# 1069066484/PanoSwinTransformerObjectDetection

Hardware: AMD Instinct MI355X
Metric: panoramas/sec PanoSwin-T 512x1024 fwd+bwd (higher is better)
Workload: dtype bf16; 1 GPU; PanoSwin-T backbone (embed 96, depths 2-2-6-2, heads 3-6-12-24, ape, pano mode) fwd+bwd+AdamW on 3x512x1024 panoramas, BASELINE.json configs[1]; batch_per_gpu=8, global_batch=8, parallelism=dp1, hip_graph=True, overlap_allreduce=False, fused_window_attention=True, device=AMD Radeon Graphics

## Files before the change

include/pswin.h:

```cpp
#ifndef PSWIN_H_
#define PSWIN_H_

#include <stdint.h>

#ifdef __cplusplus
extern "C" {
#endif

#define PSWIN_ABI_VERSION 10

#define PSWIN_F32 0
#define PSWIN_BF16 1

#define PSWIN_MODE_PLANAR 0
#define PSWIN_MODE_PANO 1

#define PSWIN_OK 0
#define PSWIN_ERR_ARG (-1)
#define PSWIN_ERR_UNSUPPORTED (-2)

#define PSWIN_WS 7
#define PSWIN_WTOK 49
#define PSWIN_WPAD 64
#define PSWIN_HEAD_DIM 32

int pswin_version(void);


int pswin_window_grid(int mode, int H, int W, int* Hp, int* Wp, int* n_windows);

int pswin_window_map(int mode, int H, int W, int shift, int32_t* map, int32_t* inv, void* stream);

int pswin_planar_mask(int H, int W, int shift, float* mask, void* stream);


int pswin_uv_grid(int H, int W, float* uv, void* stream);

int pswin_abs_pos_features(const float* uv, int n, float* feat, void* stream);

int pswin_gather_uv(const float* uv, const int32_t* map, int n_slots, float* uv_win, void* stream);

int pswin_haversine_windows(const float* uv1, const float* uv2, int n_windows, float* dist, void* stream);
// ... 259 lines not shown
                              int P, int C, void* stream);



int pswin_attn_pad_tiles(const float* src, int n, int transpose, float* dst, void* stream);

int pswin_attn_fwd(const void* q, const void* k, const void* v, int ld_qkv, const float* dist_tiles, int n_dist,
                   const float* alpha, const float* beta, const float* mask_tiles, int n_mask, void* out, int ld_out,
                   float* lse, int n_chunks, int n_windows, int n_bias_windows, int heads, float scale, int dtype,
                   void* stream);

int pswin_attn_suggest_chunks(int n_windows, int n_bias_windows, int heads, int backward);

int pswin_win_attn_fused_supported(int C, int heads, int dtype);
int pswin_win_attn_fused_fwd(const void* x, const void* w_qkv, const float* b_qkv, const void* w_proj, const float* dist_tiles,
                             int n_dist, const float* alpha, const float* beta, const float* mask_tiles, int n_mask, void* y,
                             void* qkv_out, void* att_out, float* lse_out, long long n_windows, int n_bias_windows, int C,
                             int heads, float scale, int dtype, void* stream);

int pswin_qkv_attn_fused_supported(int C, int heads, int dtype);
int pswin_qkv_attn_fused_fwd(const void* x, const void* w_qkv, const float* b_qkv, const float* dist_tiles, int n_dist, const float* alpha,
                             const float* beta, const float* mask_tiles, int n_mask, void* y, void* qkv_out, float* lse_out, long long n_windows,
                             int n_bias_windows, int C, int heads, float scale, int dtype, void* stream);

int pswin_attn_bwd(const void* q, const void* k, const void* v, int ld_qkv, const float* dist_tiles_t, int n_dist,
                   const float* alpha, const float* beta, const float* mask_tiles_t, int n_mask, const void* dout,
                   int ld_out, const float* lse, void* dq, void* dk, void* dv, int ld_dqkv, float* dscore_sum,
                   int n_chunks, int n_windows, int n_bias_windows, int heads, float scale, int dtype, void* stream);
int pswin_attn_bwd_ex(const void* q, const void* k, const void* v, int ld_qkv, long long qkv_window_stride, int qkv_head_stride,
                      const float* dist_tiles_t, int n_dist, const float* alpha, const float* beta, const float* mask_tiles_t,
                      int n_mask, const void* dout, int ld_out, const float* lse, void* dq, void* dk, void* dv, int ld_dqkv,
                      float* dscore_sum, int n_chunks, int n_windows, int n_bias_windows, int heads, float scale, int dtype,
                      void* stream);


int pswin_attn_table_grads_workspace(int heads);
int pswin_attn_table_grads_partial_rows(int n_tiles, int heads);
int pswin_attn_table_grads(const float* dscore_sum, int n_tiles, int n_bias_windows, const float* dist_tiles_t,
                           int n_dist, int heads, float* dalpha, float* dbeta, float* workspace, void* stream);

typedef struct pswin_table_grad_job {
    const float* dscore_sum;
    const float* dist_tiles_t;
    float* dalpha;
    float* dbeta;
    float* workspace;
    int n_tiles;
    int n_bias_windows;
    int n_dist;
    int heads;
} pswin_table_grad_job;
int pswin_attn_table_grads_batch(const pswin_table_grad_job* jobs, int n_jobs, int stages, void* stream);


int pswin_pano_warp_u8(const uint8_t* src, const double* params, uint8_t* dst, int B, int H, int W, int C, void* stream);

int pswin_pano_resize_normalize_pad(const uint8_t* src, const int32_t* out_hw, const float* norm, int to_rgb, float* dst, int B, int H,
                                    int W, int Hp, int Wp, void* stream);

int pswin_pano_resize_crop_resize_normalize_pad(const uint8_t* src, const int32_t* plan, const float* norm, int to_rgb, float* dst, int B,
                                                int H, int W, int Hp, int Wp, void* stream);

int pswin_pano_masks(const uint8_t* src, const double* params, const int32_t* plan, const int32_t* rows, const int32_t* count, uint8_t* dst,
                     int B, int Gin, int Gmax, int H, int W, int Hp, int Wp, void* stream);


// ... 138 lines not shown
```

panoswintransformerobjectdetection_amd/_lib.py:

```python
import ctypes
import os

import torch

_PKG = os.path.dirname(os.path.abspath(__file__))
LIB_PATH = os.environ.get("PSWIN_LIB") or os.path.join(_PKG, "libpswin_hip.so")

F32, BF16 = 0, 1
MODE_PLANAR, MODE_PANO = 0, 1
WS, WTOK, WPAD, HEAD_DIM = 7, 49, 64, 32
ABI_VERSION = 10

_vp, _i, _f = ctypes.c_void_p, ctypes.c_int, ctypes.c_float
_ip = ctypes.POINTER(ctypes.c_int)

_PROTOTYPES = {
    "pswin_version": [],
    "pswin_window_grid": [_i, _i, _i, _ip, _ip, _ip],
    "pswin_window_map": [_i, _i, _i, _i, _vp, _vp, _vp],
    "pswin_planar_mask": [_i, _i, _i, _vp, _vp],
    "pswin_uv_grid": [_i, _i, _vp, _vp],
    "pswin_abs_pos_features": [_vp, _i, _vp, _vp],
    "pswin_gather_uv": [_vp, _vp, _i, _vp, _vp],
    "pswin_haversine_windows": [_vp, _vp, _i, _vp, _vp],
    "pswin_window_gather": [_vp, _i, _vp, _vp, _vp, _i, _i, _i, _i, _i, _vp],
    "pswin_window_scatter_add": [_vp, _i, _vp, _vp, _vp, _vp, _vp, _i, _i, _i, _i, _i, _vp],
    "pswin_ln_gather_fwd": [_vp, _i, _vp, _vp, _vp, _f, _vp, _i, _vp, _vp, _i, _i, _i, _i, _vp],
    "pswin_ln_gather_fwd_add": [_vp, _i, _vp, _vp, _vp, _f, _vp, _vp, _i, _vp, _vp, _i, _i, _i, _i, _vp],
    "pswin_ln_gather_bwd": [_vp, _i, _vp, _vp, _i, _vp, _vp, _vp, _vp, _vp, _vp, _vp, _vp, _vp, _vp, _i, _i, _i, _i, _vp],
    "pswin_ln_gather_bwd_ex": [_vp, _i, _vp, _vp, _i, _vp, _vp, _vp, _vp, _vp, _vp, _vp, _vp, _vp, _vp, _i, _i, _i, _i, _vp, _vp, _i, _vp, _vp, _i,
                               _vp],
    "pswin_scatter_add_ln_fwd": [_vp, _i, _vp, _vp, _vp, _vp, _vp, _vp, _vp, _f, _vp, _i, _vp, _vp, _i, _i, _i, _i, _vp],
    "pswin_scatter_add_ln_fwd_map": [_vp, _i, _vp, _vp, _vp, _vp, _vp, _vp, _vp, _f, _vp, _i, _vp, _vp, _i, _i, _i, _i, _vp, _i, _vp, _i, _vp],
    "pswin_ln_nchw_supported": [_i, _i],
    "pswin_ln_nchw_fwd": [_vp, _vp, _vp, _f, _vp, _vp, _vp, _i, _i, _i, _vp],
    "pswin_ln_nchw_bwd": [_vp, _vp, _vp, _vp, _vp, _vp, _vp, _vp, _vp, _vp, _i, _i, _i, _vp],
    "pswin_scatter_add_ln_nchw_fwd": [_vp, _vp, _vp, _vp, _vp, _vp, _vp, _f, _vp, _vp, _vp, _i, _i, _i, _vp],
    "pswin_ln_nchw_bwd_ex": [_vp, _vp, _vp, _vp, _vp, _vp, _vp, _vp, _vp, _vp, _vp, _vp, _i, _i, _i, _vp],
    "pswin_ln_workspace": [ctypes.c_longlong, _i],
    "pswin_ln_patch_merge_fwd": [_vp, _i, _vp, _vp, _f, _vp, _i, _vp, _vp, _i, _i, _i, _i, _vp],
    "pswin_ln_patch_merge_bwd": [_vp, _i, _vp, _i, _vp, _vp, _vp, _vp, _vp, _vp, _vp, _i, _i, _i, _i, _vp],
    "pswin_patch_merge_gather": [_vp, _i, _vp, _i, _i, _i, _i, _i, _vp],
    "pswin_patch_merge_scatter": [_vp, _i, _vp, _i, _i, _i, _i, _i, _vp],
    "pswin_bn_workspace": [_i],
# ... 100 lines not shown
    "pswin_mlp0_fwd": [_vp, _vp, _vp, _vp, _vp, _vp, ctypes.c_longlong, _i, _i, _vp],
    "pswin_mlp0_bwd_supported": [_i, _i],
    "pswin_mlp0_bwd_partial_rows": [ctypes.c_longlong],
    "pswin_mlp0_bwd": [_vp, _vp, _vp, _vp, _vp, _vp, _vp, _vp, ctypes.c_longlong, _i, _i, _vp],
    "pswin_fc1_gelu_bwd": [_vp, _vp, _vp, _vp, _vp, _vp, _vp, ctypes.c_longlong, _i, _i, _vp],
    "pswin_bias_gelu_fwd": [_vp, _i, _vp, _vp, ctypes.c_longlong, _i, _vp],
    "pswin_bias_gelu_workspace": [ctypes.c_longlong, _i],
    "pswin_bias_gelu_tune": [_i, _i],
    "pswin_bias_gelu_bwd": [_vp, _vp, _i, _vp, _vp, _vp, _vp, ctypes.c_longlong, _i, _vp],
    "pswin_colsum_workspace": [ctypes.c_longlong, _i, _i],
    "pswin_colsum": [_vp, _i, ctypes.c_longlong, _i, _vp, _vp, _vp],
    "pswin_colsum_skip": [_vp, _i, ctypes.c_longlong, _i, _i, _i, _vp, _vp],
    "pswin_reduce_jobs": [_vp, _i, _vp],
    "pswin_attn_table_grads_batch": [_vp, _i, _i, _vp],
    "pswin_attn_table_grads_partial_rows": [_i, _i],
    "pswin_ln_partial_rows": [ctypes.c_longlong, _i],
    "pswin_ln_rows_tune": [_i],
    "pswin_bias_gelu_partial_rows": [ctypes.c_longlong, _i, _i],
    "pswin_fc1_gelu_partial_rows": [ctypes.c_longlong],
    "pswin_interp_rows": [_vp, _vp, _vp, _vp, _i, _i, _i, _i, _vp],
    "pswin_interp_rows_adjoint": [_vp, _vp, _vp, _vp, _i, _i, _i, _i, _vp],
    "pswin_attn_pad_tiles": [_vp, _i, _i, _vp, _vp],
    "pswin_attn_fwd": [_vp, _vp, _vp, _i, _vp, _i, _vp, _vp, _vp, _i, _vp, _i, _vp, _i, _i, _i, _i, _f, _i, _vp],
    "pswin_win_attn_fused_supported": [_i, _i, _i],
    "pswin_win_attn_fused_fwd": [_vp, _vp, _vp, _vp, _vp, _i, _vp, _vp, _vp, _i, _vp, _vp, _vp, _vp, ctypes.c_longlong, _i, _i, _i,
                                 _f, _i, _vp],
    "pswin_qkv_attn_fused_supported": [_i, _i, _i],
    "pswin_qkv_attn_fused_fwd": [_vp, _vp, _vp, _vp, _i, _vp, _vp, _vp, _i, _vp, _vp, _vp, ctypes.c_longlong, _i, _i, _i, _f, _i, _vp],
    "pswin_attn_suggest_chunks": [_i, _i, _i, _i],
    "pswin_attn_bwd": [_vp, _vp, _vp, _i, _vp, _i, _vp, _vp, _vp, _i, _vp, _i, _vp, _vp, _vp, _vp, _i, _vp,
                       _i, _i, _i, _i, _f, _i, _vp],
    "pswin_attn_bwd_ex": [_vp, _vp, _vp, _i, ctypes.c_longlong, _i, _vp, _i, _vp, _vp, _vp, _i, _vp, _i, _vp, _vp, _vp, _vp, _i, _vp,
                          _i, _i, _i, _i, _f, _i, _vp],
    "pswin_attn_table_grads_workspace": [_i],
    "pswin_attn_table_grads": [_vp, _i, _i, _vp, _i, _i, _vp, _vp, _vp, _vp],
    "pswin_pano_warp_u8": [_vp, _vp, _vp, _i, _i, _i, _i, _vp],
    "pswin_pano_resize_normalize_pad": [_vp, _vp, _vp, _i, _vp, _i, _i, _i, _i, _i, _vp],
    "pswin_pano_resize_crop_resize_normalize_pad": [_vp, _vp, _vp, _i, _vp, _i, _i, _i, _i, _i, _vp],
    "pswin_pano_masks": [_vp, _vp, _vp, _vp, _vp, _vp, _i, _i, _i, _i, _i, _i, _i, _vp],
}

_lib = None


class PswinError(RuntimeError):
    pass


class ReduceJob(ctypes.Structure):
    _fields_ = [("src", ctypes.c_void_p), ("dst", ctypes.c_void_p), ("dtype", ctypes.c_int), ("rows", ctypes.c_int),
                ("cols", ctypes.c_int), ("ld", ctypes.c_int)]


class TnJob(ctypes.Structure):
    _fields_ = [("dy", ctypes.c_void_p), ("x", ctypes.c_void_p), ("partial", ctypes.c_void_p), ("dbias_partial", ctypes.c_void_p),
                ("M", ctypes.c_longlong), ("N", ctypes.c_int), ("K", ctypes.c_int), ("splits", ctypes.c_int), ("partial_dtype", ctypes.c_int),
                ("zero_lo", ctypes.c_int), ("zero_hi", ctypes.c_int), ("sample_scale", ctypes.c_void_p), ("rows_per_sample", ctypes.c_int)]


class TransposeJob(ctypes.Structure):
    _fields_ = [("src", ctypes.c_void_p), ("dst", ctypes.c_void_p), ("rows", ctypes.c_int), ("cols", ctypes.c_int)]


class LrSchedule(ctypes.Structure):
    _fields_ = [("policy", ctypes.c_int), ("warmup", ctypes.c_int), ("warmup_iters", ctypes.c_int), ("by_epoch", ctypes.c_int),
                ("iters_per_epoch", ctypes.c_int), ("n_milestones", ctypes.c_int), ("step_every", ctypes.c_int), ("has_min_lr", ctypes.c_int),
# ... 136 lines not shown
```

panoswintransformerobjectdetection_amd/csrc/pswin_attn.hip:

```cpp
#include <cstdlib>
#include <type_traits>

#include "pswin_attn_frag.hpp"

using namespace pswin;

namespace {

struct AttnArgs {
    const void *q, *k, *v;
    const float* dist;
    const float* mask;
    const float* alpha;
    const float* beta;
    void* out;
    const void* dout;
    float* lse;
#ifdef PSWIN_ATTN_STAMPS
    unsigned long long* stamps;
#endif
    void *dq, *dk, *dv;
    float* dtab;
    int n_dist, n_mask;
    int ld_qkv, ld_out, ld_dqkv;
    long long qkv_win_stride;
    int qkv_head_stride;
    int nb, heads, reps_per_chunk, n_items;
    float scale;
};


struct TabRaw {
    float b[3], a[3];
};
static_assert(NBINS <= 3 * 64, "three table entries per lane");
__device__ inline TabRaw tables_fetch(const AttnArgs& a, int h, int lane) {
    const __amdgpu_buffer_rsrc_t bres = __builtin_amdgcn_make_buffer_rsrc(const_cast<float*>(a.beta), 0, NBINS * a.heads * 4, 0x00020000);
    const __amdgpu_buffer_rsrc_t ares = __builtin_amdgcn_make_buffer_rsrc(const_cast<float*>(a.alpha), 0, a.dist ? NBINS * a.heads * 4 : 0, 0x00020000);
    TabRaw r;
#pragma unroll
    for (int k = 0; k < 3; ++k) {
        const int off = ((lane + 64 * k) * a.heads + h) * 4;
        r.b[k] = __builtin_bit_cast(float, __builtin_amdgcn_raw_buffer_load_b32(bres, off, 0, 0));
        r.a[k] = __builtin_bit_cast(float, __builtin_amdgcn_raw_buffer_load_b32(ares, off, 0, 0));
    }
    return r;
}
__device__ inline void tables_store(const TabRaw& r, int lane, float* tab_a, float* tab_b) {
#pragma unroll
    for (int k = 0; k < 3; ++k) {
        const int t = lane + 64 * k;
        if (t < NBINS) {
            tab_b[t] = r.b[k];
            tab_a[t] = r.a[k];
        }
// ... 332 lines not shown
            for (int dt = 0; dt < 2; ++dt) kt[dt] = lds_read_tr<DT, HD>(kimg, 32 * s + 4 * g, 16 * dt, c, g);
#pragma unroll
            for (int ti = 0; ti < 4; ++ti) {
                const Frag<DT> tf = lds_read_tr<DT, PADT>(timg, 32 * s + 4 * g, 16 * ti, c, g);
#pragma unroll
                for (int dt = 0; dt < 2; ++dt) dq[dt][ti] = mma32<DT>(kt[dt], tf, dq[dt][ti]);
            }
        }
#pragma unroll
        for (int ti = 0; ti < 4; ++ti) {
            store_row8_at<DT>(window_rsrc<DT>(a.dq, dhead0, a.ld_dqkv), dx_off[ti], g, dq[0][ti] * a.scale, dq[1][ti] * a.scale);
        }
        if constexpr (DUAL) {
            if (r + 1 < a.reps_per_chunk) cur = nxt;
        }
    }
    if (a.dtab) {
        float* gt = a.dtab + (size_t)item * (PADT * PADT);
#pragma unroll
        for (int ti = 0; ti < 4; ++ti)
#pragma unroll
            for (int tj = 0; tj < 4; ++tj)
                *reinterpret_cast<f32x4*>(gt + (16 * tj + c) * PADT + 16 * ti + 4 * g) = gsum[ti][tj];
    }
}

struct PairLds {
    static constexpr int KIMG = 64 * 64;
    static constexpr int HALF = 32 * 64;
    static constexpr int TIMG = 64 * 64;
    static constexpr int EXCH = 64 * 128;
    static constexpr int TAB = 2 * TABP * 4;
    static constexpr int BYTES = KIMG + 2 * (2 * HALF + TIMG) + 2 * EXCH + TAB;
};

__device__ inline int timg_off(int row, int unit8) {
    return row * 64 + ((unit8 ^ (((row >> 1) & 1) | (((row >> 3) & 1) << 1) | (((row >> 2) & 1) << 2))) << 3);
}
__device__ inline int exch_off(int row, int chunk16) { return row * 128 + ((chunk16 ^ (row & 7)) << 4); }

template <bool TIMG>
__device__ inline Frag<PSWIN_BF16> tr32(const char* img, int R0, int col0, int c) {
    const int q = c >> 2, p = c & 3;
    typedef __attribute__((address_space(3))) s16x4* lds_s16x4_ptr;
    const int k8 = (col0 >> 2) + p;
    const char* a0 = img + (TIMG ? timg_off(R0 + q, k8) : img32_off(R0 + q, k8 >> 1) + ((k8 & 1) << 3));
    const char* a1 = a0 + 16 * 64;
    s16x4 lo = __builtin_amdgcn_ds_read_tr16_b64_v4i16((lds_s16x4_ptr)(a0));
    s16x4 hi = __builtin_amdgcn_ds_read_tr16_b64_v4i16((lds_s16x4_ptr)(a1));
    typedef __attribute__((ext_vector_type(8))) short s16x8;
    s16x8 both = {lo[0], lo[1], lo[2], lo[3], hi[0], hi[1], hi[2], hi[3]};
    Frag<PSWIN_BF16> f;
    f.v = __builtin_bit_cast(bf16x8, both);
    return f;
}

#ifdef PSWIN_ATTN_STAMPS
#define PSWIN_STAMP(i)                                                  \
    do {                                                                \
        const unsigned long long t_ = __builtin_amdgcn_s_memtime();     \
        stamp_acc[i] += t_ - stamp_last;                                \
        stamp_last = t_;                                                \
    } while (0)
#else
#define PSWIN_STAMP(i)
#endif
__global__ __launch_bounds__(128, 2) void attn_bwd_pair_kernel(AttnArgs a) {
    constexpr int DT = PSWIN_BF16;
#ifdef PSWIN_ATTN_STAMPS
    unsigned long long stamp_acc[8] = {0, 0, 0, 0, 0, 0, 0, 0}, stamp_last = __builtin_amdgcn_s_memtime();
#endif
    __shared__ __attribute__((aligned(16))) char smem[PairLds::BYTES];
    const int w = __builtin_amdgcn_readfirstlane(threadIdx.x >> 6), lane = threadIdx.x & 63;
    const int c = lane & 15, g = lane >> 4;
    const int item = blockIdx.x;
    const int h = item % a.heads;
    const int wb = (item / a.heads) % a.nb;
    const int chunk = item / (a.heads * a.nb);
    char* kimg = smem;
    char* qimg = kimg + PairLds::KIMG + w * (2 * PairLds::HALF + PairLds::TIMG);
    char* doimg = qimg + PairLds::HALF;
    char* timg = doimg + PairLds::HALF;
    float* exch_dk = reinterpret_cast<float*>(smem + PairLds::KIMG + 2 * (2 * PairLds::HALF + PairLds::TIMG));
    float* exch_dv = exch_dk + 64 * 32;
    float* tab_a = exch_dv + 64 * 32;
    float* tab_b = tab_a + TABP;
    const float* dtile = a.dist ? a.dist + (size_t)(wb % a.n_dist) * (PADT * PADT) : nullptr;
// ... 174 lines not shown
            for (int tt = 0; tt < 2; ++tt) dq[dt][tt] = f32x4{0.f, 0.f, 0.f, 0.f};
#pragma unroll
        for (int s = 0; s < 2; ++s) {
            Frag<DT> kt[2];
#pragma unroll
            for (int dt = 0; dt < 2; ++dt) kt[dt] = tr32<false>(kimg, 32 * s + 4 * g, 16 * dt, c);
#pragma unroll
            for (int tt = 0; tt < 2; ++tt) {
                const Frag<DT> tf = tr32<true>(timg, 32 * s + 4 * g, 16 * tt, c);
#pragma unroll
                for (int dt = 0; dt < 2; ++dt) dq[dt][tt] = mma32<DT>(kt[dt], tf, dq[dt][tt]);
            }
        }
#pragma unroll
        for (int tt = 0; tt < 2; ++tt) {
            store_row8_at<DT>(window_rsrc<DT>(a.dq, dhead0, a.ld_dqkv), dq_off[tt], g, dq[0][tt] * a.scale, dq[1][tt] * a.scale);
        }
        PSWIN_STAMP(5);
        __syncthreads();
        PSWIN_STAMP(6);
    }
#ifdef PSWIN_ATTN_STAMPS
    if (a.stamps && lane == 0)
        for (int i = 0; i < 8; ++i) a.stamps[((size_t)blockIdx.x * 2 + w) * 8 + i] = stamp_acc[i];
#endif
    if (a.dtab) {
        float* gt = a.dtab + (size_t)item * (PADT * PADT);
#pragma unroll
        for (int tt = 0; tt < 2; ++tt)
#pragma unroll
            for (int tj = 0; tj < 4; ++tj)
                *reinterpret_cast<f32x4*>(gt + (16 * tj + c) * PADT + 16 * (2 * w + tt) + 4 * g) = gsum[tt][tj];
    }
}

__global__ void pad_tiles_kernel(const float* __restrict__ src, int n, int transpose, float* __restrict__ dst) {
    const size_t t = blockIdx.x;
    for (int e = threadIdx.x; e < PADT * PADT; e += blockDim.x) {
        const int r = e / PADT, col = e - r * PADT;
        float v = 0.f;
        if (r < TOK && col < TOK) v = transpose ? src[(t * TOK + col) * TOK + r] : src[(t * TOK + r) * TOK + col];
        dst[t * PADT * PADT + e] = v;
    }
}

constexpr int DTAB_BLOCKS = 128;
__host__ __device__ inline int dtab_ld(int heads) { return (heads * 2 * TOK * TOK + 3) & ~3; }
inline int dtab_blocks(int n_tiles, int heads) {
    int nb = (512 + heads - 1) / heads;
    if (nb > DTAB_BLOCKS) nb = DTAB_BLOCKS;
    if (nb < 16) nb = 16;
    return n_tiles < nb ? n_tiles : nb;
}
constexpr int DTAB_THREADS = 256;

constexpr int TJ_MAX = 32;
struct TJob {
    const float* g;
    const float* dist_t;
    float* partial;
    float* summed;
    float* dalpha;
    float* dbeta;
    int n_tiles, nb, n_dist, heads, blocks;
    int first1, first2;
};
// ... 137 lines not shown
    a.nb = n_bias_windows; a.heads = heads; a.reps_per_chunk = reps / chunks;
    a.scale = scale;
    constexpr int W = 4;
    if (dtype == PSWIN_BF16) {
        a.n_items = chunks * n_bias_windows * heads * 2;
        hipLaunchKernelGGL((attn_fwd_kernel<PSWIN_BF16, W, 2>), dim3((a.n_items + W - 1) / W), dim3(64 * W), 0,
                           (hipStream_t)stream, a);
    } else {
        a.n_items = chunks * n_bias_windows * heads;
        hipLaunchKernelGGL((attn_fwd_kernel<PSWIN_F32, W, 4>), dim3((a.n_items + W - 1) / W), dim3(64 * W), 0,
                           (hipStream_t)stream, a);
    }
    PSWIN_LAUNCH_RET();
}

extern "C" int pswin_attn_suggest_chunks(int n_windows, int n_bias_windows, int heads, int backward) {
    if (n_windows <= 0 || n_bias_windows <= 0 || heads <= 0 || n_windows % n_bias_windows) return PSWIN_ERR_ARG;
    return pick_chunks(n_windows / n_bias_windows, n_bias_windows, heads, backward != 0);
}

extern "C" int pswin_attn_table_grads_partial_rows(int n_tiles, int heads) {
    return (n_tiles > 0 && heads > 0) ? dtab_blocks(n_tiles, heads) : PSWIN_ERR_ARG;
}

extern "C" int pswin_attn_table_grads_workspace(int heads) {
    return heads > 0 ? (DTAB_BLOCKS + 1) * dtab_ld(heads) : PSWIN_ERR_ARG;
}

#ifdef PSWIN_ATTN_STAMPS
static unsigned long long* g_attn_stamps = nullptr;
extern "C" void pswin_attn_debug_stamps(unsigned long long* p) { g_attn_stamps = p; }
#endif

extern "C" int pswin_attn_bwd_ex(const void* q, const void* k, const void* v, int ld_qkv, long long qkv_window_stride,
                                 int qkv_head_stride, const float* dist_t, int n_dist, const float* alpha, const float* beta,
                                 const float* mask_t, int n_mask, const void* dout, int ld_out, const float* lse, void* dq, void* dk,
                                 void* dv, int ld_dqkv, float* dscore_sum, int n_chunks, int n_windows, int n_bias_windows,
                                 int heads, float scale, int dtype, void* stream) {
    PSWIN_CHECK_ARG(q && k && v && beta && valid_dtype(dtype) && n_windows > 0 && n_bias_windows > 0 && heads > 0);
    PSWIN_CHECK_ARG(n_windows % n_bias_windows == 0 && ld_qkv >= HD && ld_qkv % 8 == 0 && qkv_head_stride % 8 == 0 && qkv_window_stride % 8 == 0);
    PSWIN_CHECK_ARG(qkv_head_stride >= HD && qkv_window_stride >= (long long)(TOK - 1) * ld_qkv + HD);
    PSWIN_CHECK_ARG(aligned16(q) && aligned16(k) && aligned16(v) && aligned16(dist_t) && aligned16(mask_t));
    PSWIN_CHECK_ARG((long long)n_windows * qkv_window_stride < (1ll << 40));
    PSWIN_CHECK_ARG(!dist_t || (alpha && n_dist > 0 && n_bias_windows % n_dist == 0));
    PSWIN_CHECK_ARG(!mask_t || (n_mask > 0 && n_bias_windows % n_mask == 0));
    PSWIN_CHECK_ARG(dout && lse && dq && dk && dv);
    PSWIN_CHECK_ARG(aligned16(dout) && aligned16(dq) && aligned16(dk) && aligned16(dv) && aligned16(lse));
    PSWIN_CHECK_ARG(ld_out >= heads * HD && ld_out % 8 == 0 && ld_dqkv >= heads * HD && ld_dqkv % 8 == 0);
    const int reps = n_windows / n_bias_windows;
    PSWIN_CHECK_ARG(n_chunks >= 1 && n_chunks <= reps && reps % n_chunks == 0);
    PSWIN_CHECK_ARG(aligned16(dscore_sum));
    AttnArgs a = {};
    a.q = q; a.k = k; a.v = v; a.dist = dist_t; a.mask = mask_t; a.alpha = alpha; a.beta = beta;
    a.n_dist = dist_t ? n_dist : 1; a.n_mask = mask_t ? n_mask : 1;
    a.dout = dout; a.lse = const_cast<float*>(lse);
    a.dq = dq; a.dk = dk; a.dv = dv; a.dtab = dscore_sum;
#ifdef PSWIN_ATTN_STAMPS
    a.stamps = g_attn_stamps;
#endif
    a.ld_qkv = ld_qkv; a.ld_out = ld_out; a.ld_dqkv = ld_dqkv;
    a.qkv_win_stride = qkv_window_stride; a.qkv_head_stride = qkv_head_stride;
    a.nb = n_bias_windows; a.heads = heads; a.reps_per_chunk = reps / n_chunks;
    a.n_items = n_chunks * n_bias_windows * heads;
    a.scale = scale;
    if (dtype == PSWIN_BF16) {
        hipLaunchKernelGGL(attn_bwd_pair_kernel, dim3(a.n_items), dim3(128), 0, (hipStream_t)stream, a);
    } else {
        constexpr int W = 3;
        hipLaunchKernelGGL((attn_bwd_kernel<PSWIN_F32, W>), dim3((a.n_items + W - 1) / W), dim3(64 * W), 0,
                           (hipStream_t)stream, a);
    }
    PSWIN_LAUNCH_RET();
}

extern "C" int pswin_attn_bwd(const void* q, const void* k, const void* v, int ld_qkv, const float* dist_t, int n_dist,
                              const float* alpha, const float* beta, const float* mask_t, int n_mask,
                              const void* dout, int ld_out, const float* lse, void* dq, void* dk, void* dv,
                              int ld_dqkv, float* dscore_sum, int n_chunks, int n_windows, int n_bias_windows,
                              int heads, float scale, int dtype, void* stream) {
    PSWIN_CHECK_ARG(ld_qkv >= heads * HD);
    return pswin_attn_bwd_ex(q, k, v, ld_qkv, (long long)TOK * ld_qkv, HD, dist_t, n_dist, alpha, beta, mask_t, n_mask, dout, ld_out, lse,
                             dq, dk, dv, ld_dqkv, dscore_sum, n_chunks, n_windows, n_bias_windows, heads, scale, dtype, stream);
}

extern "C" int pswin_attn_table_grads_batch(const pswin_table_grad_job* jobs, int n_jobs, int stages, void* stream) {
    PSWIN_CHECK_ARG(jobs && n_jobs > 0 && (stages == 1 || stages == 2 || stages == 3 || stages == 4));
    for (int j = 0; j < n_jobs; ++j) {
        const pswin_table_grad_job& q = jobs[j];
        PSWIN_CHECK_ARG(q.dscore_sum && q.dbeta && q.workspace && q.n_tiles > 0 && q.n_bias_windows > 0 && q.heads > 0);
        PSWIN_CHECK_ARG(q.n_tiles % q.n_bias_windows == 0);
        PSWIN_CHECK_ARG(!q.dist_tiles_t || (q.dalpha && q.n_dist > 0 && q.n_bias_windows % q.n_dist == 0));
    }
    for (int at = 0; at < n_jobs; at += TJ_MAX) {
        TBatch b;
        b.n = n_jobs - at < TJ_MAX ? n_jobs - at : TJ_MAX;
        long long g1 = 0, g2 = 0;
        for (int j = 0; j < b.n; ++j) {
            const pswin_table_grad_job& q = jobs[at + j];
            TJob& t = b.job[j];
            t.g = q.dscore_sum; t.dist_t = q.dist_tiles_t; t.partial = q.workspace;
            t.summed = q.workspace + (size_t)DTAB_BLOCKS * dtab_ld(q.heads);
            t.dalpha = q.dist_tiles_t ? q.dalpha : nullptr; t.dbeta = q.dbeta;
            t.n_tiles = q.n_tiles; t.nb = q.n_bias_windows; t.n_dist = q.dist_tiles_t ? q.n_dist : 1; t.heads = q.heads;
            t.blocks = dtab_blocks(q.n_tiles, q.heads);
            t.first1 = (int)g1; t.first2 = (int)g2;
// ... 22 lines not shown
```

panoswintransformerobjectdetection_amd/grad_queue.py:

```python
import ctypes
from typing import NamedTuple, Optional

import torch

from . import _lib
from ._lib import PswinError, call, dtype_code


def _addr(t):
    return None if t is None else t.data_ptr()


class Reduction(NamedTuple):
    src: torch.Tensor
    offset: int
    dtype: int
    rows: int
    cols: int
    ld: int
    dst: torch.Tensor

    @property
    def ref(self):
        return self.src
# ... 193 lines not shown
def grad_slot(param):
    slot = getattr(param, "_grad_slot", None)
    if slot is None or not param.is_leaf or param.grad is not None or slot.device != param.device or _has_hooks(param):
        return None
    task = _graph_task_id()
    if task == -1:
        return None
    used = _slots.get(task)
    if used is None:
        used = _slots[task] = set()
        _trim(_slots)
    if slot.data_ptr() in used:
        return None
    used.add(slot.data_ptr())
    return slot


def sum_rows(src, rows, cols, ld=None, col_offset=0, out=None, owners=()):
    ld = cols if ld is None else ld
    if not src.is_contiguous():
        raise PswinError("sum_rows expects a contiguous source")
    if out is None:
        out = torch.empty(cols, dtype=torch.float32, device=src.device)
    elif out.dtype != torch.float32 or out.numel() != cols or not out.is_contiguous():
        raise PswinError("sum_rows: `out` must be a contiguous float32 buffer of `cols` elements")
    q = deferring(owners)
    if q is None:
        _launch_reductions([Reduction(src, col_offset * src.element_size(), dtype_code(src), rows, cols, ld, out)])
    else:
        q.add_reduction(src, rows, cols, out, ld=ld, offset=col_offset * src.element_size())
    return out.view(cols)


def table_gradients(gsum, dist_tiles_t, n_tiles, n_bias_windows, n_dist, heads, owners, defer_partials):
    lib = _lib.load()
    dbeta = torch.empty(169, heads, dtype=torch.float32, device=gsum.device)
    dalpha = torch.empty_like(dbeta) if dist_tiles_t is not None else None
    ws = torch.empty(lib.pswin_attn_table_grads_workspace(heads), dtype=torch.float32, device=gsum.device)
    ld = ws.numel() // 129
    partial_sums = Reduction(ws, 0, _lib.F32, lib.pswin_attn_table_grads_partial_rows(n_tiles, heads), ld, ld, ws[128 * ld:])
    q = deferring(owners)
    job = TableGrad(gsum, dist_tiles_t, dalpha, dbeta, ws, n_tiles, n_bias_windows, n_dist, heads,
                    partials_deferred=q is not None and defer_partials)
    if not job.partials_deferred:
        _launch_table_grads([job], 1)
    if q is None:
        _launch_reductions([partial_sums])
        _launch_table_grads([job], 4)
        return dalpha, dbeta
    q.add_table_gradient(job, partial_sums)
    return (None if dalpha is None else dalpha.view(169, heads)), dbeta.view(169, heads)
```

panoswintransformerobjectdetection_amd/ops.py:

```python
import ctypes
import math
import os

import torch
import torch.nn.functional as F

from . import _lib
from . import grad_queue
from ._lib import BF16, F32, MODE_PANO, MODE_PLANAR, WPAD, WTOK, PswinError, call, dtype_code, ptr
from .grad_queue import deferred_reductions_available, flush_if_pending, flush_reductions, grad_slot, set_deferred_reductions, sum_rows

_CACHE = {}
_DISABLED = {n.strip().lower() for n in os.environ.get("PSWIN_DISABLE", "").split(",") if n.strip()}


def _on(name):
    return name not in _DISABLED


FUSED_WINDOW_ATTENTION = _on("fused_window_attention")
GEMM_NT = _on("gemm_nt")
FUSED_GELU_BWD = _on("fused_gelu_bwd")
FUSED_MLP = _on("fused_mlp")
DEFER_TABLE_PARTIALS = _on("defer_table_partials")
SAMPLE_SKIP = _on("sample_skip")


def _dev_key(device):
    device = torch.device(device)
    return (device.type, device.index if device.index is not None else torch.cuda.current_device())


def clear_caches():
    _CACHE.clear()


def window_maps(pano, H, W, shift, device):
    key = ("map", bool(pano), H, W, shift, _dev_key(device))
    if key not in _CACHE:
        mode = MODE_PANO if pano else MODE_PLANAR
        _, _, nW = _lib.window_grid(mode, H, W)
        wmap = torch.empty(nW * WTOK, dtype=torch.int32, device=device)
        inv = torch.empty(H * W, dtype=torch.int32, device=device)
        call("pswin_window_map", wmap, mode, H, W, shift, ptr(wmap), ptr(inv))
        _CACHE[key] = (wmap, inv, nW)
    return _CACHE[key]


def window_pads(pano, H, W, shift, device):
    key = ("pads", bool(pano), H, W, shift, _dev_key(device))
    if key not in _CACHE:
        wmap, _, _ = window_maps(pano, H, W, shift, device)
        _CACHE[key] = torch.nonzero(wmap < 0).flatten().to(torch.int32).contiguous()
    return _CACHE[key]


def identity_map(S, device):
# ... 1160 lines not shown
                                                       ctx.nb, ctx.chunks, ctx.needs_input_grad[3] or ctx.needs_input_grad[4],
                                                       ctx.owners)
        return dx, dk, dv, dalpha, dbeta, None, None, None, None, None, None


def attention_backward(x, k, v, lse, alpha, beta, dist, mask, dout, heads, scale, nb, chunks, need_tables, owners, packed=False):
    C = heads * _lib.HEAD_DIM
    n = x.shape[0] if packed else x.shape[0] // WTOK
    fused = k is None
    dout = dout.contiguous()
    es = x.element_size()
    ld_in, win_stride, head_stride = None, None, _lib.HEAD_DIM
    if packed:
        dx = torch.empty(n * WTOK, 3 * C, dtype=x.dtype, device=x.device)
        ld = 3 * C
        blk = WTOK * _lib.HEAD_DIM
        qp, kp, vp = x.data_ptr(), x.data_ptr() + blk * es, x.data_ptr() + 2 * blk * es
        dqp, dkp, dvp = dx.data_ptr(), dx.data_ptr() + C * es, dx.data_ptr() + 2 * C * es
        dk = dv = None
        ld_in, win_stride, head_stride = _lib.HEAD_DIM, heads * 3 * blk, 3 * blk
    elif fused:
        dx = torch.empty_like(x)
        ld = 3 * C
        qp, kp, vp = x.data_ptr(), x.data_ptr() + C * es, x.data_ptr() + 2 * C * es
        dqp, dkp, dvp = dx.data_ptr(), dx.data_ptr() + C * es, dx.data_ptr() + 2 * C * es
        dk = dv = None
    else:
        dx, dk, dv = torch.empty_like(x), torch.empty_like(k), torch.empty_like(v)
        ld = C
        qp, kp, vp = x.data_ptr(), k.data_ptr(), v.data_ptr()
        dqp, dkp, dvp = dx.data_ptr(), dk.data_ptr(), dv.data_ptr()
    lib = _lib.load()
    chunks = chunks or lib.pswin_attn_suggest_chunks(n, nb, heads, 1)
    dalpha = dbeta = gsum = None
    if need_tables:
        gsum = torch.empty(chunks * nb, heads, WPAD, WPAD, dtype=torch.float32, device=x.device)
    ld_in = ld if ld_in is None else ld_in
    win_stride = WTOK * ld_in if win_stride is None else win_stride
    call("pswin_attn_bwd_ex", x, ctypes.c_void_p(qp), ctypes.c_void_p(kp), ctypes.c_void_p(vp), ld_in, win_stride, head_stride,
         ptr(None if dist is None else dist.bwd), 0 if dist is None else dist.n, ptr(alpha), ptr(beta),
         ptr(None if mask is None else mask.bwd), 0 if mask is None else mask.n, ptr(dout), C, ptr(lse),
         ctypes.c_void_p(dqp), ctypes.c_void_p(dkp), ctypes.c_void_p(dvp), ld, ptr(gsum),
         chunks, n, nb, heads, scale, dtype_code(x),
         algo_bytes=n * heads * 7 * WTOK * _lib.HEAD_DIM * x.element_size())
    if need_tables:
        dalpha, dbeta = grad_queue.table_gradients(gsum, None if dist is None else dist.bwd, chunks * nb, nb, 0 if dist is None else dist.n,
                                                   heads, owners, DEFER_TABLE_PARTIALS)
    return dx, dk, dv, dalpha, dbeta


def window_attention(qkv, alpha, beta, dist, mask, heads, scale, n_bias_windows, k=None, v=None, chunks=None):
    return _WindowAttention.apply(qkv, k, v, alpha, beta, _as_tiles(dist), _as_tiles(mask), heads, scale,
                                  n_bias_windows, chunks)


class _WindowAttentionFused(torch.autograd.Function):

    @staticmethod
    def forward(ctx, x, w_qkv, b_qkv, w_proj, alpha, beta, dist, mask, heads, scale, n_bias_windows, wq_lp, wp_lp, grad_mode):
        x = x.contiguous()
        rows, C = x.shape
        n = rows // WTOK
        assert rows % WTOK == 0 and C == heads * _lib.HEAD_DIM
        wq = (wq_lp if wq_lp is not None else w_qkv.to(x.dtype)).contiguous()
        wp = (wp_lp if wp_lp is not None else w_proj.to(x.dtype)).contiguous()
        bq = None if b_qkv is None else b_qkv.detach().float().contiguous()
        alpha_c = alpha.detach().contiguous() if dist is not None else None
        beta_c = beta.detach().contiguous()
        save = grad_mode and any(ctx.needs_input_grad)
        y = torch.empty_like(x)
        qkv = att = lse = None
        if save:
            qkv = torch.empty(n, heads, 3, WTOK, _lib.HEAD_DIM, dtype=x.dtype, device=x.device)
            att = torch.empty_like(x)
            lse = torch.empty(n, heads, WPAD, dtype=torch.float32, device=x.device)
        flops = n * (2 * WTOK * C * 3 * C + heads * 4 * WTOK * WTOK * _lib.HEAD_DIM + 2 * WTOK * C * C)
        call("pswin_win_attn_fused_fwd", x, ptr(x), ptr(wq), ptr(bq), ptr(wp), ptr(None if dist is None else dist.fwd),
             0 if dist is None else dist.n, ptr(alpha_c), ptr(beta_c), ptr(None if mask is None else mask.fwd),
# ... 854 lines not shown
```

Baseline: 881.0 panoramas/s.

## Bin relative-position table gradients inside attention backward kernel

```diff
diff --git a/include/pswin.h b/include/pswin.h
--- a/include/pswin.h
+++ b/include/pswin.h
@@ -7,7 +7,7 @@
 extern "C" {
 #endif
 
-#define PSWIN_ABI_VERSION 10
+#define PSWIN_ABI_VERSION 11
 
 #define PSWIN_F32 0
 #define PSWIN_BF16 1
@@ -333,6 +333,12 @@
                       int n_mask, const void* dout, int ld_out, const float* lse, void* dq, void* dk, void* dv, int ld_dqkv,
                       float* dscore_sum, int n_chunks, int n_windows, int n_bias_windows, int heads, float scale, int dtype,
                       void* stream);
+int pswin_attn_table_bins_ld(int heads);
+int pswin_attn_bwd_bins(const void* q, const void* k, const void* v, int ld_qkv, long long qkv_window_stride, int qkv_head_stride,
+                        const float* dist_tiles_t, int n_dist, const float* alpha, const float* beta, const float* mask_tiles_t,
+                        int n_mask, const void* dout, int ld_out, const float* lse, void* dq, void* dk, void* dv, int ld_dqkv,
+                        float* dscore_sum, float* dtab_bins, int n_chunks, int n_windows, int n_bias_windows, int heads, float scale,
+                        int dtype, void* stream);
 
 
 int pswin_attn_table_grads_workspace(int heads);
diff --git a/panoswintransformerobjectdetection_amd/_lib.py b/panoswintransformerobjectdetection_amd/_lib.py
--- a/panoswintransformerobjectdetection_amd/_lib.py
+++ b/panoswintransformerobjectdetection_amd/_lib.py
@@ -9,7 +9,7 @@
 F32, BF16 = 0, 1
 MODE_PLANAR, MODE_PANO = 0, 1
 WS, WTOK, WPAD, HEAD_DIM = 7, 49, 64, 32
-ABI_VERSION = 10
+ABI_VERSION = 11
 
 _vp, _i, _f = ctypes.c_void_p, ctypes.c_int, ctypes.c_float
 _ip = ctypes.POINTER(ctypes.c_int)
@@ -176,6 +176,9 @@
                        _i, _i, _i, _i, _f, _i, _vp],
     "pswin_attn_bwd_ex": [_vp, _vp, _vp, _i, ctypes.c_longlong, _i, _vp, _i, _vp, _vp, _vp, _i, _vp, _i, _vp, _vp, _vp, _vp, _i, _vp,
                           _i, _i, _i, _i, _f, _i, _vp],
+    "pswin_attn_table_bins_ld": [_i],
+    "pswin_attn_bwd_bins": [_vp, _vp, _vp, _i, ctypes.c_longlong, _i, _vp, _i, _vp, _vp, _vp, _i, _vp, _i, _vp, _vp, _vp, _vp, _i, _vp, _vp,
+                            _i, _i, _i, _i, _f, _i, _vp],
     "pswin_attn_table_grads_workspace": [_i],
     "pswin_attn_table_grads": [_vp, _i, _i, _vp, _i, _i, _vp, _vp, _vp, _vp],
     "pswin_pano_warp_u8": [_vp, _vp, _vp, _i, _i, _i, _i, _vp],
diff --git a/panoswintransformerobjectdetection_amd/csrc/pswin_attn.hip b/panoswintransformerobjectdetection_amd/csrc/pswin_attn.hip
--- a/panoswintransformerobjectdetection_amd/csrc/pswin_attn.hip
+++ b/panoswintransformerobjectdetection_amd/csrc/pswin_attn.hip
@@ -21,6 +21,8 @@
 #endif
     void *dq, *dk, *dv;
     float* dtab;
+    float* dbins;
+    int dbins_ld;
     int n_dist, n_mask;
     int ld_qkv, ld_out, ld_dqkv;
     long long qkv_win_stride;
@@ -419,7 +421,10 @@
     static constexpr int EXCH = 64 * 128;
     static constexpr int TAB = 2 * TABP * 4;
     static constexpr int BYTES = KIMG + 2 * (2 * HALF + TIMG) + 2 * EXCH + TAB;
+    static constexpr int BINP = 68;
+    static constexpr int BINT = 64 * BINP;
 };
+static_assert(2 * PairLds::BINT * 4 <= PairLds::BYTES - PairLds::TAB, "the two binning tiles fit below the staged tables");
 
 __device__ inline int timg_off(int row, int unit8) {
     return row * 64 + ((unit8 ^ (((row >> 1) & 1) | (((row >> 3) & 1) << 1) | (((row >> 2) & 1) << 2))) << 3);
@@ -440,6 +445,24 @@
     Frag<PSWIN_BF16> f;
     f.v = __builtin_bit_cast(bf16x8, both);
     return f;
+}
+
+template <bool ALPHA>
+__device__ inline void bin_sums(const float* gl, const float* dl, int bin, float& sb, float& sa) {
+    const int dh = bin / (2 * PSWIN_WS - 1) - (PSWIN_WS - 1), dw = bin % (2 * PSWIN_WS - 1) - (PSWIN_WS - 1);
+    const int off = PSWIN_WS * dh + dw;
+    sb = sa = 0.f;
+#pragma unroll
+    for (int hj = 0; hj < PSWIN_WS; ++hj)
+#pragma unroll
+        for (int wj = 0; wj < PSWIN_WS; ++wj) {
+            if ((unsigned)(hj + dh) < (unsigned)PSWIN_WS && (unsigned)(wj + dw) < (unsigned)PSWIN_WS) {
+                const int e = (PSWIN_WS * hj + wj) * (PairLds::BINP + 1) + off;
+                const float gv = gl[e];
+                sb += gv;
+                if (ALPHA) sa = __builtin_fmaf(gv, dl[e], sa);
+            }
+        }
 }
 
 #ifdef PSWIN_ATTN_STAMPS
@@ -680,6 +703,36 @@
             for (int tj = 0; tj < 4; ++tj)
                 *reinterpret_cast<f32x4*>(gt + (16 * tj + c) * PADT + 16 * (2 * w + tt) + 4 * g) = gsum[tt][tj];
     }
+    if (a.dbins) {
+        constexpr int BINP = PairLds::BINP;
+        float* gl = reinterpret_cast<float*>(smem);
+        float* dl = gl + PairLds::BINT;
+        const int t = threadIdx.x;
+        if (dtile) {
+            f32x4 dq4[7];
+#pragma unroll
+            for (int k = 0; k < 7; ++k) dq4[k] = *reinterpret_cast<const f32x4*>(dtile + 4 * (t + 128 * k));
+#pragma unroll
+            for (int k = 0; k < 7; ++k) {
+                const int q = t + 128 * k;
+                *reinterpret_cast<f32x4*>(dl + (q >> 4) * BINP + 4 * (q & 15)) = dq4[k];
+            }
+        }
+#pragma unroll
+        for (int tt = 0; tt < 2; ++tt)
+#pragma unroll
+            for (int tj = 0; tj < 4; ++tj)
+                *reinterpret_cast<f32x4*>(gl + (16 * tj + c) * BINP + 16 * (2 * w + tt) + 4 * g) = gsum[tt][tj];
+        __syncthreads();
+        float* row = a.dbins + (size_t)(chunk * a.nb + wb) * a.dbins_ld + h;
+        for (int bin = t; bin < NBINS; bin += 128) {
+            float sb, sa;
+            if (dtile) bin_sums<true>(gl, dl, bin, sb, sa);
+            else bin_sums<false>(gl, dl, bin, sb, sa);
+            row[(size_t)bin * a.heads] = sb;
+            if (dtile) row[(size_t)(NBINS + bin) * a.heads] = sa;
+        }
+    }
 }
 
 __global__ void pad_tiles_kernel(const float* __restrict__ src, int n, int transpose, float* __restrict__ dst) {
@@ -883,11 +936,15 @@
 extern "C" void pswin_attn_debug_stamps(unsigned long long* p) { g_attn_stamps = p; }
 #endif
 
-extern "C" int pswin_attn_bwd_ex(const void* q, const void* k, const void* v, int ld_qkv, long long qkv_window_stride,
-                                 int qkv_head_stride, const float* dist_t, int n_dist, const float* alpha, const float* beta,
-                                 const float* mask_t, int n_mask, const void* dout, int ld_out, const float* lse, void* dq, void* dk,
-                                 void* dv, int ld_dqkv, float* dscore_sum, int n_chunks, int n_windows, int n_bias_windows,
-                                 int heads, float scale, int dtype, void* stream) {
+namespace {
+
+inline int dbins_ld(int heads) { return (2 * NBINS * heads + 3) & ~3; }
+
+int attn_bwd_launch(const void* q, const void* k, const void* v, int ld_qkv, long long qkv_window_stride,
+                    int qkv_head_stride, const float* dist_t, int n_dist, const float* alpha, const float* beta,
+                    const float* mask_t, int n_mask, const void* dout, int ld_out, const float* lse, void* dq, void* dk,
+                    void* dv, int ld_dqkv, float* dscore_sum, float* dtab_bins, int n_chunks, int n_windows, int n_bias_windows,
+                    int heads, float scale, int dtype, void* stream) {
     PSWIN_CHECK_ARG(q && k && v && beta && valid_dtype(dtype) && n_windows > 0 && n_bias_windows > 0 && heads > 0);
     PSWIN_CHECK_ARG(n_windows % n_bias_windows == 0 && ld_qkv >= HD && ld_qkv % 8 == 0 && qkv_head_stride % 8 == 0 && qkv_window_stride % 8 == 0);
     PSWIN_CHECK_ARG(qkv_head_stride >= HD && qkv_window_stride >= (long long)(TOK - 1) * ld_qkv + HD);
@@ -900,12 +957,14 @@
     PSWIN_CHECK_ARG(ld_out >= heads * HD && ld_out % 8 == 0 && ld_dqkv >= heads * HD && ld_dqkv % 8 == 0);
     const int reps = n_windows / n_bias_windows;
     PSWIN_CHECK_ARG(n_chunks >= 1 && n_chunks <= reps && reps % n_chunks == 0);
-    PSWIN_CHECK_ARG(aligned16(dscore_sum));
+    PSWIN_CHECK_ARG(aligned16(dscore_sum) && aligned16(dtab_bins));
+    if (dtab_bins && dtype != PSWIN_BF16) return PSWIN_ERR_UNSUPPORTED;
     AttnArgs a = {};
     a.q = q; a.k = k; a.v = v; a.dist = dist_t; a.mask = mask_t; a.alpha = alpha; a.beta = beta;
     a.n_dist = dist_t ? n_dist : 1; a.n_mask = mask_t ? n_mask : 1;
     a.dout = dout; a.lse = const_cast<float*>(lse);
     a.dq = dq; a.dk = dk; a.dv = dv; a.dtab = dscore_sum;
+    a.dbins = dtab_bins; a.dbins_ld = dbins_ld(heads);
 #ifdef PSWIN_ATTN_STAMPS
     a.stamps = g_attn_stamps;
 #endif
@@ -922,6 +981,28 @@
                            (hipStream_t)stream, a);
     }
     PSWIN_LAUNCH_RET();
+}
+
+}
+
+extern "C" int pswin_attn_bwd_ex(const void* q, const void* k, const void* v, int ld_qkv, long long qkv_window_stride,
+                                 int qkv_head_stride, const float* dist_t, int n_dist, const float* alpha, const float* beta,
+                                 const float* mask_t, int n_mask, const void* dout, int ld_out, const float* lse, void* dq, void* dk,
+                                 void* dv, int ld_dqkv, float* dscore_sum, int n_chunks, int n_windows, int n_bias_windows,
+                                 int heads, float scale, int dtype, void* stream) {
+    return attn_bwd_launch(q, k, v, ld_qkv, qkv_window_stride, qkv_head_stride, dist_t, n_dist, alpha, beta, mask_t, n_mask, dout, ld_out,
+                           lse, dq, dk, dv, ld_dqkv, dscore_sum, nullptr, n_chunks, n_windows, n_bias_windows, heads, scale, dtype, stream);
+}
+
+extern "C" int pswin_attn_table_bins_ld(int heads) { return heads > 0 ? dbins_ld(heads) : PSWIN_ERR_ARG; }
+
+extern "C" int pswin_attn_bwd_bins(const void* q, const void* k, const void* v, int ld_qkv, long long qkv_window_stride,
+                                   int qkv_head_stride, const float* dist_t, int n_dist, const float* alpha, const float* beta,
+                                   const float* mask_t, int n_mask, const void* dout, int ld_out, const float* lse, void* dq, void* dk,
+                                   void* dv, int ld_dqkv, float* dscore_sum, float* dtab_bins, int n_chunks, int n_windows,
+                                   int n_bias_windows, int heads, float scale, int dtype, void* stream) {
+    return attn_bwd_launch(q, k, v, ld_qkv, qkv_window_stride, qkv_head_stride, dist_t, n_dist, alpha, beta, mask_t, n_mask, dout, ld_out,
+                           lse, dq, dk, dv, ld_dqkv, dscore_sum, dtab_bins, n_chunks, n_windows, n_bias_windows, heads, scale, dtype, stream);
 }
 
 extern "C" int pswin_attn_bwd(const void* q, const void* k, const void* v, int ld_qkv, const float* dist_t, int n_dist,
diff --git a/panoswintransformerobjectdetection_amd/grad_queue.py b/panoswintransformerobjectdetection_amd/grad_queue.py
--- a/panoswintransformerobjectdetection_amd/grad_queue.py
+++ b/panoswintransformerobjectdetection_amd/grad_queue.py
@@ -249,6 +249,24 @@
     return out.view(cols)
 
 
+def table_bins_ld(heads):
+    return _lib.load().pswin_attn_table_bins_ld(heads)
+
+
+def table_bin_gradients(bins, has_dist, heads, owners):
+    n = 169 * heads
+    rows, ld = bins.shape
+    cols = ld if has_dist else (n + 3) & ~3
+    out = torch.empty(cols, dtype=torch.float32, device=bins.device)
+    job = Reduction(bins, 0, _lib.F32, rows, cols, ld, out)
+    q = deferring(owners)
+    if q is None:
+        _launch_reductions([job])
+    else:
+        q.reductions.append(job)
+    return (out[n:2 * n].view(169, heads) if has_dist else None), out[:n].view(169, heads)
+
+
 def table_gradients(gsum, dist_tiles_t, n_tiles, n_bias_windows, n_dist, heads, owners, defer_partials):
     lib = _lib.load()
     dbeta = torch.empty(169, heads, dtype=torch.float32, device=gsum.device)
diff --git a/panoswintransformerobjectdetection_amd/ops.py b/panoswintransformerobjectdetection_amd/ops.py
--- a/panoswintransformerobjectdetection_amd/ops.py
+++ b/panoswintransformerobjectdetection_amd/ops.py
@@ -23,6 +23,7 @@
 FUSED_GELU_BWD = _on("fused_gelu_bwd")
 FUSED_MLP = _on("fused_mlp")
 DEFER_TABLE_PARTIALS = _on("defer_table_partials")
+TABLE_BINS = _on("table_bins")
 SAMPLE_SKIP = _on("sample_skip")
 
 
@@ -1249,18 +1250,24 @@
         dqp, dkp, dvp = dx.data_ptr(), dk.data_ptr(), dv.data_ptr()
     lib = _lib.load()
     chunks = chunks or lib.pswin_attn_suggest_chunks(n, nb, heads, 1)
-    dalpha = dbeta = gsum = None
-    if need_tables:
+    dalpha = dbeta = gsum = bins = None
+    if need_tables and TABLE_BINS and x.dtype == torch.bfloat16:
+        bins = torch.empty(chunks * nb, grad_queue.table_bins_ld(heads), dtype=torch.float32, device=x.device)
+    elif need_tables:
         gsum = torch.empty(chunks * nb, heads, WPAD, WPAD, dtype=torch.float32, device=x.device)
     ld_in = ld if ld_in is None else ld_in
     win_stride = WTOK * ld_in if win_stride is None else win_stride
-    call("pswin_attn_bwd_ex", x, ctypes.c_void_p(qp), ctypes.c_void_p(kp), ctypes.c_void_p(vp), ld_in, win_stride, head_stride,
+    tables_out = (ptr(gsum),) if bins is None else (None, ptr(bins))
+    call("pswin_attn_bwd_ex" if bins is None else "pswin_attn_bwd_bins", x, ctypes.c_void_p(qp), ctypes.c_void_p(kp), ctypes.c_void_p(vp),
+         ld_in, win_stride, head_stride,
          ptr(None if dist is None else dist.bwd), 0 if dist is None else dist.n, ptr(alpha), ptr(beta),
          ptr(None if mask is None else mask.bwd), 0 if mask is None else mask.n, ptr(dout), C, ptr(lse),
-         ctypes.c_void_p(dqp), ctypes.c_void_p(dkp), ctypes.c_void_p(dvp), ld, ptr(gsum),
+         ctypes.c_void_p(dqp), ctypes.c_void_p(dkp), ctypes.c_void_p(dvp), ld, *tables_out,
          chunks, n, nb, heads, scale, dtype_code(x),
-         algo_bytes=n * heads * 7 * WTOK * _lib.HEAD_DIM * x.element_size())
-    if need_tables:
+         algo_bytes=n * heads * 7 * WTOK * _lib.HEAD_DIM * x.element_size(), timed_as="pswin_attn_bwd_ex")
+    if bins is not None:
+        dalpha, dbeta = grad_queue.table_bin_gradients(bins, dist is not None, heads, owners)
+    elif need_tables:
         dalpha, dbeta = grad_queue.table_gradients(gsum, None if dist is None else dist.bwd, chunks * nb, nb, 0 if dist is None else dist.n,
                                                    heads, owners, DEFER_TABLE_PARTIALS)
     return dx, dk, dv, dalpha, dbeta
```

Result: no change. 889.1 panoramas/s (median of 6 runs) (+0.9%).
